# cxy1997/3D_adapt_auto_driving

Measured on AMD Instinct MI355X. Metric: KITTI scenes/s end-to-end eval_rcnn (joint RPN+RCNN, synthetic 16384-pt scenes), higher is better.
Workload: dtype f32; 1 GPU; BASELINE.json configs[2]: full PointRCNN RPN+RCNN inference, default.yaml shapes, random-init weights, batch=8 synthetic KITTI scenes x 16384 pts per GPU per step; scene=synth.scenes (SURVEY 8d: uniform clutter + ground + 10 dense cars), parallelism=scene-sharded x1, one final all_gather of detections, detections_gathered=652455, batch_slots=14, look_ahead=12, steps_per_launch=2

## Files before the change

### 3d_adapt_auto_driving_amd/csrc/fps_spec.hip

```cpp
#include "fps_common.hpp"
#include <stdlib.h>
#include <map>
#include <mutex>

namespace prcnn {



constexpr int FS_RMAX = 16;

__device__ __forceinline__ float fs_shfl(float v, int src, int wbase)
{
    const int index = (src & (WAVE - 1)) + wbase;
    return __int_as_float(__builtin_amdgcn_ds_bpermute(index << 2, __float_as_int(v)));
}

template <int PPT, int I = 0>
__device__ __forceinline__ void fs_pick3(const float (&px)[PPT], const float (&py)[PPT], const float (&pz)[PPT], int slot, int l,
                                         float &x, float &y, float &z)
{
    if (slot == I) {
        x = __int_as_float(__builtin_amdgcn_readlane(__float_as_int(px[I]), l));
        y = __int_as_float(__builtin_amdgcn_readlane(__float_as_int(py[I]), l));
        z = __int_as_float(__builtin_amdgcn_readlane(__float_as_int(pz[I]), l));
    } else if constexpr (I + 1 < PPT) {
        fs_pick3<PPT, I + 1>(px, py, pz, slot, l, x, y, z);
    }
}

template <int PPT>
__global__ __launch_bounds__(1024) void fps_spec_kernel(
    int n, int m, KeyCodec kc, const float *__restrict__ xyz, const int *__restrict__ perm,
    float *__restrict__ temp, int *__restrict__ idx, float *__restrict__ new_xyz, const int *__restrict__ rejected = nullptr)
{
    constexpr int SB = PPT == 16 ? 4 : (PPT == 8 ? 3 : 2);
    __shared__ unsigned long long s_vk[32];
    __shared__ float s_xyz[32][3];
    __shared__ float s_bound[16];
    __shared__ int s_rank[32], s_blk[32];
    const int b = blockIdx.x;
    if (rejected && rejected[b] == 0) return;
    const float *__restrict__ cloud = xyz + (long)b * n * 3;
    const int *__restrict__ order = perm + (long)b * n;
    float *__restrict__ mind = temp ? temp + (long)b * n : nullptr;
    int *__restrict__ sel = idx + (long)b * m;
    float *__restrict__ nxyz = new_xyz ? new_xyz + (long)b * m * 3 : nullptr;
    const int t = threadIdx.x, lane = t & 63, w = t >> 6;
    __builtin_amdgcn_s_setprio(3);

    float px[PPT], py[PPT], pz[PPT], pt[PPT];
    uint32_t pc[PPT];
    float bx0 = INFINITY, bx1 = -INFINITY, by0 = INFINITY, by1 = -INFINITY, bz0 = INFINITY, bz1 = -INFINITY;
#pragma unroll
    for (int i = 0; i < PPT; ++i) {
        const int s = w * (64 * PPT) + i * 64 + lane;
        float x0 = INFINITY, x1 = -INFINITY, y0 = INFINITY, y1 = -INFINITY, z0 = INFINITY, z1 = -INFINITY;
        if (s < n) {
            const int k = order[s];
            px[i] = cloud[3 * k]; py[i] = cloud[3 * k + 1]; pz[i] = cloud[3 * k + 2];
            pt[i] = mind ? mind[k] : 1e10f;
            pc[i] = (kc.encode(k) << SB) | (uint32_t)i;
            x0 = x1 = px[i]; y0 = y1 = py[i]; z0 = z1 = pz[i];
        } else {
            px[i] = py[i] = pz[i] = 0.f;
            pt[i] = -INFINITY;
            pc[i] = 0xffffffffu;
        }
#pragma unroll
        for (int d = 32; d >= 1; d >>= 1) {
            x0 = fmin_raw(x0, __shfl_xor(x0, d, 64)); x1 = fmax_raw(x1, __shfl_xor(x1, d, 64));
            y0 = fmin_raw(y0, __shfl_xor(y0, d, 64)); y1 = fmax_raw(y1, __shfl_xor(y1, d, 64));
            z0 = fmin_raw(z0, __shfl_xor(z0, d, 64)); z1 = fmax_raw(z1, __shfl_xor(z1, d, 64));
        }
        if (lane == i) { bx0 = x0; bx1 = x1; by0 = y0; by1 = y1; bz0 = z0; bz1 = z1; }
    }

    constexpr int GP = 64 / PPT;
    const int wbase = (int)__lane_id() & ~(WAVE - 1);
    bx0 = fs_shfl(bx0, lane & (PPT - 1), wbase); bx1 = fs_shfl(bx1, lane & (PPT - 1), wbase);
    by0 = fs_shfl(by0, lane & (PPT - 1), wbase); by1 = fs_shfl(by1, lane & (PPT - 1), wbase);
    bz0 = fs_shfl(bz0, lane & (PPT - 1), wbase); bz1 = fs_shfl(bz1, lane & (PPT - 1), wbase);
    unsigned long long touched = 0ull, etiles = ~0ull;
    float bound = INFINITY;
    auto box_mask = [&](float ox, float oy, float oz, bool live) __attribute__((always_inline)) {
        const float dx = fmax_raw(fmax_raw(bx0 - ox, ox - bx1), 0.f);
        const float dy = fmax_raw(fmax_raw(by0 - oy, oy - by1), 0.f);
        const float dz = fmax_raw(fmax_raw(bz0 - oz, oz - bz1), 0.f);
        const float lb = dx * dx + dy * dy + dz * dz;
        return __ballot(live && !(lb * 0.99999f >= bound));
    };
    auto update = [&](float ox, float oy, float oz, unsigned long long mask) __attribute__((always_inline)) {
        if (mask != 0ull) {
            touched |= mask & etiles;
            const pk_f32x2 o_x = {ox, ox}, o_y = {oy, oy}, o_z = {oz, oz};
            if (kc.hipcc) {
#pragma unroll
                for (int i = 0; i < PPT; i += 2)
                    if ((mask >> i) & 3ull) {
                        const pk_f32x2 dx = (pk_f32x2){px[i], px[i + 1]} - o_x, dy = (pk_f32x2){py[i], py[i + 1]} - o_y,
                                       dz = (pk_f32x2){pz[i], pz[i + 1]} - o_z;
                        const pk_f32x2 d = __builtin_elementwise_fma(dy, dy, dx * dx) + dz * dz;
                        pt[i] = fmin_raw(d.x, pt[i]); pt[i + 1] = fmin_raw(d.y, pt[i + 1]);
                    }
            } else {
#pragma unroll
                for (int i = 0; i < PPT; i += 2)
                    if ((mask >> i) & 3ull) {
                        const pk_f32x2 dx = (pk_f32x2){px[i], px[i + 1]} - o_x, dy = (pk_f32x2){py[i], py[i + 1]} - o_y,
                                       dz = (pk_f32x2){pz[i], pz[i + 1]} - o_z;
                        const pk_f32x2 d = (dx * dx + dy * dy) + dz * dz;
                        pt[i] = fmin_raw(d.x, pt[i]); pt[i + 1] = fmin_raw(d.y, pt[i + 1]);
                    }
            }
        }
    };
    if (t == 0) {
        sel[0] = 0;
        if (nxyz) { nxyz[0] = cloud[0]; nxyz[1] = cloud[1]; nxyz[2] = cloud[2]; }
    }
    if (t < 32) { s_rank[t] = 0; s_blk[t] = 0; }
    int j = 1;
    if (m > 1) {
        const float ox = cloud[0], oy = cloud[1], oz = cloud[2];
        update(ox, oy, oz, box_mask(ox, oy, oz, lane < PPT));
    }
    touched = ~0ull;
    while (j < m) {
        if (touched != 0ull) {
            float bv = -INFINITY, sv = -INFINITY;
#pragma unroll
            for (int i = 0; i < PPT; ++i) {
                sv = __builtin_amdgcn_fmed3f(bv, sv, pt[i]);
                bv = fmax_raw(bv, pt[i]);
            }
            uint32_t lk = 0xffffffffu;
#pragma unroll
            for (int i = 0; i < PPT; ++i) {
                const uint32_t c = pt[i] == bv ? pc[i] : 0xffffffffu;
                lk = c < lk ? c : lk;
            }
            const float v1 = wave_max_f32(bv);
            const uint32_t c1 = wave_min_u32(bv == v1 ? lk : 0xffffffffu);
            const unsigned long long m1 = __ballot(bv == v1 && lk == c1);
            const int l1 = m1 ? (int)__builtin_ctzll(m1) : 0;
            const float bv2 = lane == l1 ? -INFINITY : bv;
            const float v2 = wave_max_f32(bv2);
            const uint32_t c2 = wave_min_u32(bv2 == v2 ? lk : 0xffffffffu);
            const unsigned long long m2 = __ballot(lane != l1 && bv2 == v2 && lk == c2);
            const int l2 = m2 ? (int)__builtin_ctzll(m2) : l1;
            const float v3 = wave_max_f32((lane == l1 || lane == l2) ? -INFINITY : bv);
            const float s1 = __int_as_float(__builtin_amdgcn_readlane(__float_as_int(sv), l1));
            const float s2 = __int_as_float(__builtin_amdgcn_readlane(__float_as_int(sv), l2));
            const float wB = fmax_raw(v3, fmax_raw(s1, s2));
            bound = v1;
            const int sl1 = (int)(c1 & ((1u << SB) - 1u)), sl2 = (int)(c2 & ((1u << SB) - 1u));
            const bool has2 = m2 != 0ull && c2 != 0xffffffffu;
            etiles = (1ull << sl1) | (has2 ? (1ull << sl2) : 0ull);
            float x1 = 0.f, y1 = 0.f, z1 = 0.f, x2 = 0.f, y2 = 0.f, z2 = 0.f;
            fs_pick3<PPT>(px, py, pz, __builtin_amdgcn_readfirstlane(sl1), l1, x1, y1, z1);
            fs_pick3<PPT>(px, py, pz, __builtin_amdgcn_readfirstlane(sl2), l2, x2, y2, z2);
            const float ex = lane == 0 ? x1 : x2, ey = lane == 0 ? y1 : y2, ez = lane == 0 ? z1 : z2;
            if (lane < 2) {
                const float ev = lane == 0 ? v1 : (has2 ? v2 : -INFINITY);
                const uint32_t ek = lane == 0 ? (c1 == 0xffffffffu ? 0xffffffffu : (c1 >> SB)) : (has2 ? (c2 >> SB) : 0xffffffffu);
                s_vk[2 * w + lane] = pack_candidate(ev, ek);
                s_xyz[2 * w + lane][0] = ex; s_xyz[2 * w + lane][1] = ey; s_xyz[2 * w + lane][2] = ez;
                if (lane == 0) s_bound[w] = wB;
            }
        }
        lds_barrier();
        const int left = m - j;
        const int e = lane & 31, h = lane >> 5;
        const unsigned long long pke = s_vk[e];
        float cv; uint32_t ck;
        unpack_candidate(pke, cv, ck);
        const float cx = s_xyz[e][0], cy = s_xyz[e][1], cz = s_xyz[e][2];
        const float gB = wave_max_f32(lane < 16 ? s_bound[lane] : -INFINITY);
        {
            const int i = 2 * w + h;
            const unsigned long long pki = s_vk[i];
            float iv; uint32_t ik;
            unpack_candidate(pki, iv, ik);
            const float ix = s_xyz[i][0], iy = s_xyz[i][1], iz = s_xyz[i][2];
            const bool before = pke > pki;
            const float d = kc.hipcc ? fps_dist<true>(ix, iy, iz, cx, cy, cz) : sqdist3(ix, iy, iz, cx, cy, cz);
            const unsigned long long bb = __ballot(before), kb = __ballot(before && (d < iv));
            if (e == 0) {
                s_rank[i] = __popc((unsigned)(h ? (bb >> 32) : bb));
                s_blk[i] = (unsigned)(h ? (kb >> 32) : kb) != 0u;
            }
        }
        lds_barrier();
        const int rank = s_rank[e];
        const bool blocked = s_blk[e] != 0;
        const bool valid = !(ck == 0xffffffffu || !(cv > -1.0f));
        const bool pass = rank == 0 ? true : ((cv > gB) && (cv > 0.f) && valid && !blocked);
        const bool stop = !pass || (rank == 0 && !valid);
        int r = (int)wave_min_u32((stop && !(rank == 0)) ? (uint32_t)rank : ((rank == 0 && !valid) ? 1u : 32u));
        r = min(min(r, left), FS_RMAX);
        if (r < 1) r = 1;
        const float ox_ = valid ? cx : cloud[0], oy_ = valid ? cy : cloud[1], oz_ = valid ? cz : cloud[2];
        if (w == 0 && h == 0 && rank < r) {
            sel[j + rank] = valid ? kc.decode(ck) : 0;
            if (nxyz) { nxyz[3 * (j + rank)] = ox_; nxyz[3 * (j + rank) + 1] = oy_; nxyz[3 * (j + rank) + 2] = oz_; }
        }
        const int dst = (h == 0 && rank < FS_RMAX) ? 3 * rank : 63;
        const float rv = __int_as_float(__builtin_amdgcn_ds_permute(dst << 2, __float_as_int(ox_)) |
                                        __builtin_amdgcn_ds_permute(min(dst + 1, 63) << 2, __float_as_int(oy_)) |
                                        __builtin_amdgcn_ds_permute(min(dst + 2, 63) << 2, __float_as_int(oz_)));
        j += r;
        const int apply_n = j >= m ? r - 1 : r;
        touched = 0ull;
        for (int q0 = 0; q0 < apply_n; q0 += GP) {
            const int qg = q0 + lane / PPT;
            const int src = 3 * min(qg, FS_RMAX - 1);
            const float gx = fs_shfl(rv, src, wbase), gy = fs_shfl(rv, src + 1, wbase), gz = fs_shfl(rv, src + 2, wbase);
            const unsigned long long masks = box_mask(gx, gy, gz, qg < apply_n);
            if (masks == 0ull) continue;
#pragma unroll
            for (int g = 0; g < GP; ++g) {
                const unsigned long long mk = (masks >> (g * PPT)) & ((PPT == 64) ? ~0ull : ((1ull << PPT) - 1ull));
                if (mk != 0ull) {
                    const int q = q0 + g;
                    const float ox = __int_as_float(__builtin_amdgcn_readlane(__float_as_int(rv), 3 * q));
                    const float oy = __int_as_float(__builtin_amdgcn_readlane(__float_as_int(rv), 3 * q + 1));
                    const float oz = __int_as_float(__builtin_amdgcn_readlane(__float_as_int(rv), 3 * q + 2));
                    update(ox, oy, oz, mk);
                }
            }
        }
    }
    if (mind) {
#pragma unroll
        for (int i = 0; i < PPT; ++i)
            if (pc[i] != 0xffffffffu) mind[kc.decode(pc[i] >> SB)] = pt[i];
    }
}

struct Fps2Table {
    unsigned long long vk[2][64];
    float xyz[2][64][4];
    float bound[2][32];
    unsigned int sync;
    unsigned int pad[63];
};

__device__ __forceinline__ unsigned long long ld_agent_u64(const unsigned long long *p)
{
    return __hip_atomic_load(p, __ATOMIC_RELAXED, __HIP_MEMORY_SCOPE_AGENT);
}
__device__ __forceinline__ float ld_agent_f32(const float *p)
{
    return __int_as_float(__hip_atomic_load(reinterpret_cast<const int *>(p), __ATOMIC_RELAXED, __HIP_MEMORY_SCOPE_AGENT));
}

__device__ __forceinline__ void st_agent_u64(unsigned long long *p, unsigned long long v)
{
    __hip_atomic_store(p, v, __ATOMIC_RELAXED, __HIP_MEMORY_SCOPE_AGENT);
}
__device__ __forceinline__ void st_agent_f32(float *p, float v)
{
    __hip_atomic_store(reinterpret_cast<int *>(p), __float_as_int(v), __ATOMIC_RELAXED, __HIP_MEMORY_SCOPE_AGENT);
}

__global__ __launch_bounds__(1024) void fps_spec2_kernel(
    int nclouds, int n, int m, KeyCodec kc, const float *__restrict__ xyz, const int *__restrict__ perm,
    float *__restrict__ temp, int *__restrict__ idx, float *__restrict__ new_xyz, Fps2Table *__restrict__ tables)
{
    constexpr int PPT = 16, SB = 4, NE = 64;
    __shared__ unsigned long long s_vk[NE];
    __shared__ float s_xyz[NE][3];
    __shared__ float s_bound[32];
    __shared__ float s_res[64];
    __shared__ int s_rank[NE], s_blk[NE];
    __shared__ unsigned long long s_evk[32];
    __shared__ float s_exyz[32][3], s_eb[16];
    const int q_ = blockIdx.x;
    const int b = (q_ >> 4) * 8 + (q_ & 7), half = (q_ >> 3) & 1;
    if (b >= nclouds) return;
    const float *__restrict__ cloud = xyz + (long)b * n * 3;
    const int *__restrict__ order = perm + (long)b * n;
    float *__restrict__ mind = temp ? temp + (long)b * n : nullptr;
    int *__restrict__ sel = idx + (long)b * m;
    float *__restrict__ nxyz = new_xyz ? new_xyz + (long)b * m * 3 : nullptr;
    Fps2Table *__restrict__ tb = tables + b;
    const int t = threadIdx.x, lane = t & 63, w = t >> 6, gw = 16 * half + w;
    __builtin_amdgcn_s_setprio(3);

    float px[PPT], py[PPT], pz[PPT], pt[PPT];
    uint32_t pc[PPT];
    float bx0 = INFINITY, bx1 = -INFINITY, by0 = INFINITY, by1 = -INFINITY, bz0 = INFINITY, bz1 = -INFINITY;
#pragma unroll
    for (int i = 0; i < PPT; ++i) {
        const int s = gw * (64 * PPT) + i * 64 + lane;
        float x0 = INFINITY, x1 = -INFINITY, y0 = INFINITY, y1 = -INFINITY, z0 = INFINITY, z1 = -INFINITY;
        if (s < n) {
            const int k = order[s];
            px[i] = cloud[3 * k]; py[i] = cloud[3 * k + 1]; pz[i] = cloud[3 * k + 2];
            pt[i] = mind ? mind[k] : 1e10f;
            pc[i] = (kc.encode(k) << SB) | (uint32_t)i;
            x0 = x1 = px[i]; y0 = y1 = py[i]; z0 = z1 = pz[i];
        } else {
            px[i] = py[i] = pz[i] = 0.f;
            pt[i] = -INFINITY;
            pc[i] = 0xffffffffu;
        }
#pragma unroll
        for (int d = 32; d >= 1; d >>= 1) {
            x0 = fmin_raw(x0, __shfl_xor(x0, d, 64)); x1 = fmax_raw(x1, __shfl_xor(x1, d, 64));
            y0 = fmin_raw(y0, __shfl_xor(y0, d, 64)); y1 = fmax_raw(y1, __shfl_xor(y1, d, 64));
            z0 = fmin_raw(z0, __shfl_xor(z0, d, 64)); z1 = fmax_raw(z1, __shfl_xor(z1, d, 64));
        }
        if (lane == i) { bx0 = x0; bx1 = x1; by0 = y0; by1 = y1; bz0 = z0; bz1 = z1; }
    }
    constexpr int GP = 64 / PPT;
    const int wbase = (int)__lane_id() & ~(WAVE - 1);
    bx0 = fs_shfl(bx0, lane & (PPT - 1), wbase); bx1 = fs_shfl(bx1, lane & (PPT - 1), wbase);
    by0 = fs_shfl(by0, lane & (PPT - 1), wbase); by1 = fs_shfl(by1, lane & (PPT - 1), wbase);
    bz0 = fs_shfl(bz0, lane & (PPT - 1), wbase); bz1 = fs_shfl(bz1, lane & (PPT - 1), wbase);
    unsigned long long touched = 0ull;
    float bound = INFINITY;
    auto box_mask = [&](float ox, float oy, float oz, bool live) __attribute__((always_inline)) {
        const float dx = fmax_raw(fmax_raw(bx0 - ox, ox - bx1), 0.f);
        const float dy = fmax_raw(fmax_raw(by0 - oy, oy - by1), 0.f);
        const float dz = fmax_raw(fmax_raw(bz0 - oz, oz - bz1), 0.f);
        const float lb = dx * dx + dy * dy + dz * dz;
        return __ballot(live && !(lb * 0.99999f >= bound));
    };
    auto update = [&](float ox, float oy, float oz, unsigned long long mask) __attribute__((always_inline)) {
        if (mask != 0ull) {
            touched |= mask;
            const pk_f32x2 o_x = {ox, ox}, o_y = {oy, oy}, o_z = {oz, oz};
            if (kc.hipcc) {
#pragma unroll
                for (int i = 0; i < PPT; i += 2)
                    if ((mask >> i) & 3ull) {
                        const pk_f32x2 dx = (pk_f32x2){px[i], px[i + 1]} - o_x, dy = (pk_f32x2){py[i], py[i + 1]} - o_y,
                                       dz = (pk_f32x2){pz[i], pz[i + 1]} - o_z;
                        const pk_f32x2 d = __builtin_elementwise_fma(dy, dy, dx * dx) + dz * dz;
                        pt[i] = fmin_raw(d.x, pt[i]); pt[i + 1] = fmin_raw(d.y, pt[i + 1]);
                    }
            } else {
#pragma unroll
                for (int i = 0; i < PPT; i += 2)
                    if ((mask >> i) & 3ull) {
                        const pk_f32x2 dx = (pk_f32x2){px[i], px[i + 1]} - o_x, dy = (pk_f32x2){py[i], py[i + 1]} - o_y,
                                       dz = (pk_f32x2){pz[i], pz[i + 1]} - o_z;
                        const pk_f32x2 d = (dx * dx + dy * dy) + dz * dz;
                        pt[i] = fmin_raw(d.x, pt[i]); pt[i + 1] = fmin_raw(d.y, pt[i + 1]);
                    }
            }
        }
    };
    if (t == 0 && half == 0) {
        sel[0] = 0;
        if (nxyz) { nxyz[0] = cloud[0]; nxyz[1] = cloud[1]; nxyz[2] = cloud[2]; }
    }
    if (t < NE) { s_rank[t] = 0; s_blk[t] = 0; }
    int j = 1;
    if (m > 1) {
        const float ox = cloud[0], oy = cloud[1], oz = cloud[2];
        update(ox, oy, oz, box_mask(ox, oy, oz, lane < PPT));
    }
    touched = ~0ull;
    unsigned int round = 0;
    while (j < m) {
        if (touched != 0ull) {
            float bv = -INFINITY, sv = -INFINITY;
#pragma unroll
            for (int i = 0; i < PPT; ++i) {
                sv = __builtin_amdgcn_fmed3f(bv, sv, pt[i]);
                bv = fmax_raw(bv, pt[i]);
            }
            uint32_t lk = 0xffffffffu;
#pragma unroll
            for (int i = 0; i < PPT; ++i) {
                const uint32_t c = pt[i] == bv ? pc[i] : 0xffffffffu;
                lk = c < lk ? c : lk;
            }
            const float v1 = wave_max_f32(bv);
            const uint32_t c1 = wave_min_u32(bv == v1 ? lk : 0xffffffffu);
            const unsigned long long m1 = __ballot(bv == v1 && lk == c1);
            const int l1 = m1 ? (int)__builtin_ctzll(m1) : 0;
            const float bv2 = lane == l1 ? -INFINITY : bv;
            const float v2 = wave_max_f32(bv2);
            const uint32_t c2 = wave_min_u32(bv2 == v2 ? lk : 0xffffffffu);
            const unsigned long long m2 = __ballot(lane != l1 && bv2 == v2 && lk == c2);
            const int l2 = m2 ? (int)__builtin_ctzll(m2) : l1;
            const float v3 = wave_max_f32((lane == l1 || lane == l2) ? -INFINITY : bv);
            const float s1 = __int_as_float(__builtin_amdgcn_readlane(__float_as_int(sv), l1));
            const float s2 = __int_as_float(__builtin_amdgcn_readlane(__float_as_int(sv), l2));
            const float e_b = fmax_raw(v3, fmax_raw(s1, s2));
            bound = v1;
            const int sl1 = (int)(c1 & ((1u << SB) - 1u)), sl2 = (int)(c2 & ((1u << SB) - 1u));
            const bool has2 = m2 != 0ull && c2 != 0xffffffffu;
            float x1 = 0.f, y1 = 0.f, z1 = 0.f, x2 = 0.f, y2 = 0.f, z2 = 0.f;
            fs_pick3<PPT>(px, py, pz, __builtin_amdgcn_readfirstlane(sl1), l1, x1, y1, z1);
            fs_pick3<PPT>(px, py, pz, __builtin_amdgcn_readfirstlane(sl2), l2, x2, y2, z2);
            const float ev = lane == 0 ? v1 : (has2 ? v2 : -INFINITY);
            const uint32_t ek = lane == 0 ? (c1 == 0xffffffffu ? 0xffffffffu : (c1 >> SB)) : (has2 ? (c2 >> SB) : 0xffffffffu);
            if (lane < 2) {
                s_evk[2 * w + lane] = pack_candidate(ev, ek);
                s_exyz[2 * w + lane][0] = lane == 0 ? x1 : x2; s_exyz[2 * w + lane][1] = lane == 0 ? y1 : y2; s_exyz[2 * w + lane][2] = lane == 0 ? z1 : z2;
                if (lane == 0) s_eb[w] = e_b;
            }
        }
        const int par = (int)(round & 1u);
        if (lane < 2) {
            const int e = 2 * gw + lane, le = 2 * w + lane;
            st_agent_u64(&tb->vk[par][e], s_evk[le]);
            st_agent_f32(&tb->xyz[par][e][0], s_exyz[le][0]); st_agent_f32(&tb->xyz[par][e][1], s_exyz[le][1]);
            st_agent_f32(&tb->xyz[par][e][2], s_exyz[le][2]);
            if (lane == 0) st_agent_f32(&tb->bound[par][gw], s_eb[w]);
        }
        asm volatile("s_waitcnt vmcnt(0)" ::: "memory");
        __syncthreads();
        if (t == 0) {
            __hip_atomic_fetch_add(&tb->sync, 1u, __ATOMIC_RELEASE, __HIP_MEMORY_SCOPE_AGENT);
            const unsigned int want = 2u * (round + 1u);
            const long long t0 = wall_clock64();
            while (__hip_atomic_load(&tb->sync, __ATOMIC_ACQUIRE, __HIP_MEMORY_SCOPE_AGENT) < want) {
                __builtin_amdgcn_s_sleep(1);
                if (wall_clock64() - t0 > 400000000ll) __builtin_trap();
            }
        }
        __syncthreads();
        if (t < NE) {
            s_vk[t] = ld_agent_u64(&tb->vk[par][t]);
            s_xyz[t][0] = ld_agent_f32(&tb->xyz[par][t][0]);
            s_xyz[t][1] = ld_agent_f32(&tb->xyz[par][t][1]);
            s_xyz[t][2] = ld_agent_f32(&tb->xyz[par][t][2]);
            if (t < 32) s_bound[t] = ld_agent_f32(&tb->bound[par][t]);
        }
        __syncthreads();
        const int left = m - j;
        const int i = lane;
        const unsigned long long pki = s_vk[i];
        float cv; uint32_t ck;
        unpack_candidate(pki, cv, ck);
        const float cx = s_xyz[i][0], cy = s_xyz[i][1], cz = s_xyz[i][2];
        {
            int rk = 0;
            bool bl = false;
#pragma unroll 1
            for (int u = 0; u < 4; ++u) {
                const int e = 4 * w + u;
                const unsigned long long pke = s_vk[e];
                const float ex = s_xyz[e][0], ey = s_xyz[e][1], ez = s_xyz[e][2];
                const bool before = pke > pki;
                const float d = kc.hipcc ? fps_dist<true>(cx, cy, cz, ex, ey, ez) : sqdist3(cx, cy, cz, ex, ey, ez);
                rk += before ? 1 : 0;
                bl = bl || (before && (d < cv));
            }
            if (rk) atomicAdd(&s_rank[i], rk);
            if (bl) atomicOr(&s_blk[i], 1);
        }
        lds_barrier();
        if (w == 0) {
            const int rank = s_rank[i];
            const bool blocked = s_blk[i] != 0;
            const float gB = wave_max_f32(lane < 32 ? s_bound[lane] : -INFINITY);
            const bool valid = !(ck == 0xffffffffu || !(cv > -1.0f));
            const bool pass = rank == 0 ? true : ((cv > gB) && (cv > 0.f) && valid && !blocked);
            const bool stop = !pass || (rank == 0 && !valid);
            int r = (int)wave_min_u32((stop && !(rank == 0)) ? (uint32_t)rank : ((rank == 0 && !valid) ? 1u : 64u));
            r = min(min(r, left), FS_RMAX);
            if (r < 1) r = 1;
            if (rank < r) {
                const bool v0 = valid;
                const float ox = v0 ? cx : cloud[0], oy = v0 ? cy : cloud[1], oz = v0 ? cz : cloud[2];
                s_res[1 + 3 * rank] = ox; s_res[2 + 3 * rank] = oy; s_res[3 + 3 * rank] = oz;
                if (half == 0) {
                    sel[j + rank] = valid ? kc.decode(ck) : 0;
                    if (nxyz) { nxyz[3 * (j + rank)] = ox; nxyz[3 * (j + rank) + 1] = oy; nxyz[3 * (j + rank) + 2] = oz; }
                }
            }
            s_rank[i] = 0; s_blk[i] = 0;
            if (lane == 0) s_res[0] = __int_as_float(r);
        }
        lds_barrier();
        const float rv = s_res[lane];
        const int r = __builtin_amdgcn_readfirstlane(__float_as_int(rv));
        j += r;
        const int apply_n = j >= m ? r - 1 : r;
        touched = 0ull;
        for (int q0 = 0; q0 < apply_n; q0 += GP) {
            const int qg = q0 + lane / PPT;
            const int src = 1 + 3 * min(qg, FS_RMAX - 1);
            const float gx = fs_shfl(rv, src, wbase), gy = fs_shfl(rv, src + 1, wbase), gz = fs_shfl(rv, src + 2, wbase);
            const unsigned long long masks = box_mask(gx, gy, gz, qg < apply_n);
            if (masks == 0ull) continue;
#pragma unroll
            for (int g = 0; g < GP; ++g) {
                const unsigned long long mk = (masks >> (g * PPT)) & ((1ull << PPT) - 1ull);
                if (mk != 0ull) {
                    const int q = q0 + g;
                    const float ox = __int_as_float(__builtin_amdgcn_readlane(__float_as_int(rv), 1 + 3 * q));
                    const float oy = __int_as_float(__builtin_amdgcn_readlane(__float_as_int(rv), 2 + 3 * q));
                    const float oz = __int_as_float(__builtin_amdgcn_readlane(__float_as_int(rv), 3 + 3 * q));
                    update(ox, oy, oz, mk);
                }
            }
        }
        ++round;
    }
    if (mind) {
#pragma unroll
        for (int i = 0; i < PPT; ++i)
            if (pc[i] != 0xffffffffu) mind[kc.decode(pc[i] >> SB)] = pt[i];
    }
}

static size_t fps_lds_pad()
{
    static const size_t pad = (size_t)(getenv("PRCNN_FPS_LDS_PAD") ? atoi(getenv("PRCNN_FPS_LDS_PAD")) : 84) * 1024;
    return pad;
}

int fps2_capacity()
{
    static std::mutex mu;
    static std::map<int, int> cache;
    const size_t pad = fps_lds_pad();
    int dev = 0;
    if (hipGetDevice(&dev) != hipSuccess) { (void)hipGetLastError(); return 0; }
    std::lock_guard<std::mutex> lock(mu);
    auto it = cache.find(dev);
    if (it != cache.end()) return it->second;
    int cap = 0, per_cu = 0, cus = 0;
    if (ensure_dynamic_lds((const void *)prcnn::fps_spec2_kernel, pad, "furthest_point_sampling(two workgroups)") == PRCNN_OK &&
        hipOccupancyMaxActiveBlocksPerMultiprocessor(&per_cu, (const void *)prcnn::fps_spec2_kernel, 1024, pad) == hipSuccess &&
        hipDeviceGetAttribute(&cus, hipDeviceAttributeMultiprocessorCount, dev) == hipSuccess)
        cap = per_cu * cus;
    else
        (void)hipGetLastError();
    if (const char *e = getenv("PRCNN_FPS2_CAPACITY")) cap = atoi(e);
    cache[dev] = cap;
    return cap;
}

int launch_fps_spec2(int b, int n, int m, KeyCodec kc, const float *xyz, float *temp, int *idx, float *new_xyz, hipStream_t st)
{
    int *perm = (int *)scratch_for(st, (size_t)b * n * sizeof(int), 1);
    Fps2Table *tables = (Fps2Table *)scratch_for(st, (size_t)b * sizeof(Fps2Table), 13);
    if (!perm || !tables) { set_error("fps: cannot allocate the ordering / exchange scratch"); return PRCNN_ELAUNCH; }
    launch_fps_order(b, n, xyz, perm, nullptr, st);
    if (hipMemsetAsync(tables, 0, (size_t)b * sizeof(Fps2Table), st) != hipSuccess) {
        (void)hipGetLastError();
        set_error("fps: cannot reset the exchange tables");
        return PRCNN_ELAUNCH;
    }
    const int per = (fps2_capacity() / 2 / 16) * 8;
    for (int off = 0; off < b; off += per) {
        const int nb = b - off < per ? b - off : per;
        const unsigned grid = (unsigned)((nb + 7) / 8) * 16u;
        hipLaunchKernelGGL(fps_spec2_kernel, dim3(grid), dim3(1024), fps_lds_pad(), st, nb, n, m, kc, xyz + (size_t)off * n * 3, perm + (size_t)off * n,
                           temp ? temp + (size_t)off * n : nullptr, idx + (size_t)off * m, new_xyz ? new_xyz + (size_t)off * m * 3 : nullptr,
                           tables + off);
    }
    return check_launch("furthest_point_sampling(two workgroups)");
}

int launch_fps_spec(int b, int n, int m, KeyCodec kc, const float *xyz, float *temp, int *idx, float *new_xyz, const int *rejected, hipStream_t st)
{
    int *perm = (int *)scratch_for(st, (size_t)b * n * sizeof(int), 1);
    if (!perm) { set_error("fps: cannot allocate ordering scratch"); return PRCNN_ELAUNCH; }
    launch_fps_order(b, n, xyz, perm, rejected, st);
    const size_t pad = b <= 128 ? fps_lds_pad() : 0;
    const void *ss[3] = {(const void *)fps_spec_kernel<4>, (const void *)fps_spec_kernel<8>, (const void *)fps_spec_kernel<16>};
    if (pad)
        for (const void *k : ss) {
            const int rc = ensure_dynamic_lds(k, pad, "furthest_point_sampling(speculative)");
            if (rc != PRCNN_OK) return rc;
        }
    if (n <= 4096) hipLaunchKernelGGL((fps_spec_kernel<4>), dim3(b), dim3(1024), pad, st, n, m, kc, xyz, perm, temp, idx, new_xyz, rejected);
    else if (n <= 8192) hipLaunchKernelGGL((fps_spec_kernel<8>), dim3(b), dim3(1024), pad, st, n, m, kc, xyz, perm, temp, idx, new_xyz, rejected);
    else hipLaunchKernelGGL((fps_spec_kernel<16>), dim3(b), dim3(1024), pad, st, n, m, kc, xyz, perm, temp, idx, new_xyz, rejected);
    return check_launch("furthest_point_sampling(speculative)");
}

}
```

### profiles/fps_stamps.py

```python
import ctypes, importlib, os, subprocess, sys
import numpy as np

ROOT = os.path.dirname(os.path.dirname(os.path.abspath(__file__)))
CSRC = os.path.join(ROOT, "3d_adapt_auto_driving_amd", "csrc")
EXP = os.path.join(ROOT, "profiles", "_exp")
LIB = os.path.join(EXP, "libprcnn_hip_fps_stamps.so")
FLAGS = "--offload-arch=gfx950 -O3 -std=c++17 -fPIC -ffp-contract=off -fno-fast-math".split()
NPH = 8


def instrument():
    s = open(os.path.join(CSRC, "fps_spec.hip")).read()
    s = s.replace('#include "fps_common.hpp"', '#include "%s/fps_common.hpp"' % CSRC)
    a = s.index("template <int PPT>\n__global__ __launch_bounds__(1024) void fps_spec_kernel(")
    b = s.index("// The speculative kernel for 16384 < n <= 32768")
    k = s[a:b]

    def put(old, new):
        nonlocal k
        assert k.count(old) == 1, old[:70]
        k = k.replace(old, new)
    put("    while (j < m) {\n", "    unsigned long long acc_[%d] = {0}, t_prev_ = __builtin_amdgcn_s_memtime();\n#define PH(i) { const unsigned long long n_ = __builtin_amdgcn_s_memtime(); acc_[i] += n_ - t_prev_; t_prev_ = n_; }\n    while (j < m) {\n        acc_[7] += 1;\n" % NPH)
    put("        lds_barrier();                                                // A: the table is complete\n", "        PH(0)\n        lds_barrier();                                                // A: the table is complete\n        PH(1)\n")
    put("        lds_barrier();                                                // A2: every entry has its rank\n", "        PH(2)\n        lds_barrier();                                                // A2: every entry has its rank\n        PH(3)\n")
    put("        // ---- 4. running minima against this round's pivots (the last pick of the whole run does not update them: sampling_gpu.cu)\n", "        PH(4)\n        PH(5)\n        // ---- 4. running minima against this round's pivots (the last pick of the whole run does not update them: sampling_gpu.cu)\n")
    put("    if (mind) {\n#pragma unroll\n        for (int i = 0; i < PPT; ++i)\n            if (pc[i] != 0xffffffffu) mind[kc.decode(pc[i] >> SB)] = pt[i];\n    }\n}",
        "    if (mind) {\n#pragma unroll\n        for (int i = 0; i < PPT; ++i)\n            if (pc[i] != 0xffffffffu) mind[kc.decode(pc[i] >> SB)] = pt[i];\n    }\n"
        "    if (blockIdx.x == 0 && lane == 0) for (int i = 0; i < %d; ++i) g_fps_acc[w * %d + i] = acc_[i];\n}" % (NPH, NPH))
    put("                    update(ox, oy, oz, mk);\n                }\n            }\n        }\n    }\n", "                    update(ox, oy, oz, mk);\n                }\n            }\n        }\n        PH(6)\n    }\n")
    k = "__device__ unsigned long long g_fps_acc[16 * %d];\n" % NPH + k
    s = s[:a] + k + s[b:]
    s += ('\nextern "C" int prcnn_debug_fps_acc(unsigned long long *dst)\n{\n    return (int)hipMemcpyFromSymbol(dst, HIP_SYMBOL(prcnn::g_fps_acc), '
          'sizeof(unsigned long long) * 16 * %d);\n}\n' % NPH)
    return s


def build():
    os.makedirs(EXP, exist_ok=True)
    subprocess.check_call(["make", "-C", CSRC])
    src = os.path.join(EXP, "fps_stamps.hip")
    open(src, "w").write(instrument())
    obj = os.path.join(EXP, "fps_stamps.o")
    subprocess.check_call(["/opt/rocm/bin/hipcc"] + FLAGS + ["-c", src, "-o", obj])
    objs = [os.path.join(CSRC, "build", f) for f in sorted(os.listdir(os.path.join(CSRC, "build"))) if f.endswith(".o") and f != "fps_spec.o"]
    subprocess.check_call(["/opt/rocm/bin/hipcc", "--offload-arch=gfx950", "-shared", "-fPIC", "-o", LIB, obj] + objs)
    print("built", LIB)


def run(kind):
    import torch
    sys.path.insert(0, ROOT)
    L = importlib.import_module("3d_adapt_auto_driving_amd._lib")
    L.LIB_PATH = LIB
    pkg = importlib.import_module("3d_adapt_auto_driving_amd"); sys.path.insert(0, pkg.DROPIN_DIR)
    import pointnet2_cuda as P
    synth = importlib.import_module("3d_adapt_auto_driving_amd.synth")
    dev = torch.device("cuda", 0)
    xyz = torch.from_numpy((synth.lidar_scenes if kind == "lidar" else synth.scenes)(8, 16384, seed0=0)).to(dev)
    n, m = 16384, 4096
    temp = torch.empty((8, n), device=dev); idx = torch.empty((8, m), dtype=torch.int32, device=dev)
    for _ in range(3):
        temp.fill_(1e10); P.furthest_point_sampling_wrapper(8, n, m, xyz, temp, idx)
    torch.cuda.synchronize()
    buf = (ctypes.c_ulonglong * (16 * NPH))()
    lib = ctypes.CDLL(LIB)
    assert lib.prcnn_debug_fps_acc(buf) == 0
    a = np.array(buf, dtype=np.float64).reshape(16, NPH)
    rounds = a[:, 7]
    print("%s scenes, cloud 0, 16384 -> 4096: %d rounds; s_memtime cycles per round by wave" % (kind, int(rounds[0])))
    print("wave | rebuild+publish | wait A | pairs | wait A2 | verdict + permute (every wave, round 6) | - | updates | sum")
    for w in range(16):
        v = a[w, :7] / rounds[w]
        print("%4d | " % w + " | ".join("%7.1f" % x for x in v) + " | %7.1f" % v.sum())
    v = (a[:, :7] / rounds[:, None]).mean(0)
    print("mean | " + " | ".join("%7.1f" % x for x in v) + " | %7.1f" % v.sum())


if __name__ == "__main__":
    if sys.argv[1] == "build":
        build()
    else:
        run(sys.argv[2] if len(sys.argv) > 2 else "uniform")
```

Before: 9047 scenes/s.

## Cull FPS pivot updates with per-wave bounding box and drop permute broadcasts

Each wave now keeps a bounding box over all its points and tests every accepted pivot against it. Only pivots that could lower some running minimum in the wave are iterated, serially, and each is read with readlane or a uniform LDS load. This replaces the ds_permute/bpermute broadcast and the grouped per-tile box tests. It also adds a fast path in the key tie-break that skips a wave-min reduction when exactly one lane holds the maximum, and turns the slot pick into a binary search. The risk is that serial per-pivot iteration is slower when most pivots hit the wave.

```diff
diff --git a/3d_adapt_auto_driving_amd/csrc/fps_spec.hip b/3d_adapt_auto_driving_amd/csrc/fps_spec.hip
--- a/3d_adapt_auto_driving_amd/csrc/fps_spec.hip
+++ b/3d_adapt_auto_driving_amd/csrc/fps_spec.hip
@@ -9,22 +9,33 @@
 
 constexpr int FS_RMAX = 16;
 
-__device__ __forceinline__ float fs_shfl(float v, int src, int wbase)
-{
-    const int index = (src & (WAVE - 1)) + wbase;
-    return __int_as_float(__builtin_amdgcn_ds_bpermute(index << 2, __float_as_int(v)));
-}
-
-template <int PPT, int I = 0>
+__device__ __forceinline__ float fs_uniform(float v)
+{
+    return __int_as_float(__builtin_amdgcn_readfirstlane(__float_as_int(v)));
+}
+__device__ __forceinline__ float fs_readlane(float v, int l)
+{
+    return __int_as_float(__builtin_amdgcn_readlane(__float_as_int(v), l));
+}
+
+__device__ __forceinline__ void fs_key_of(bool in, bool also, uint32_t lk, uint32_t &c, unsigned long long &m)
+{
+    const unsigned long long a = __ballot(in);
+    if (__popcll(a) == 1) c = (uint32_t)__builtin_amdgcn_readlane((int)lk, (int)__builtin_ctzll(a));
+    else c = wave_min_u32(in ? lk : 0xffffffffu);
+    m = a & __ballot(also && lk == c);
+}
+
+template <int PPT, int LO = 0, int N = PPT>
 __device__ __forceinline__ void fs_pick3(const float (&px)[PPT], const float (&py)[PPT], const float (&pz)[PPT], int slot, int l,
                                          float &x, float &y, float &z)
 {
-    if (slot == I) {
-        x = __int_as_float(__builtin_amdgcn_readlane(__float_as_int(px[I]), l));
-        y = __int_as_float(__builtin_amdgcn_readlane(__float_as_int(py[I]), l));
-        z = __int_as_float(__builtin_amdgcn_readlane(__float_as_int(pz[I]), l));
-    } else if constexpr (I + 1 < PPT) {
-        fs_pick3<PPT, I + 1>(px, py, pz, slot, l, x, y, z);
+    if constexpr (N == 1) {
+        x = fs_readlane(px[LO], l); y = fs_readlane(py[LO], l); z = fs_readlane(pz[LO], l);
+    } else if (slot < LO + N / 2) {
+        fs_pick3<PPT, LO, N / 2>(px, py, pz, slot, l, x, y, z);
+    } else {
+        fs_pick3<PPT, LO + N / 2, N / 2>(px, py, pz, slot, l, x, y, z);
     }
 }
 
@@ -51,6 +62,7 @@
     float px[PPT], py[PPT], pz[PPT], pt[PPT];
     uint32_t pc[PPT];
     float bx0 = INFINITY, bx1 = -INFINITY, by0 = INFINITY, by1 = -INFINITY, bz0 = INFINITY, bz1 = -INFINITY;
+    float wx0 = INFINITY, wx1 = -INFINITY, wy0 = INFINITY, wy1 = -INFINITY, wz0 = INFINITY, wz1 = -INFINITY;
 #pragma unroll
     for (int i = 0; i < PPT; ++i) {
         const int s = w * (64 * PPT) + i * 64 + lane;
@@ -73,13 +85,11 @@
             z0 = fmin_raw(z0, __shfl_xor(z0, d, 64)); z1 = fmax_raw(z1, __shfl_xor(z1, d, 64));
         }
         if (lane == i) { bx0 = x0; bx1 = x1; by0 = y0; by1 = y1; bz0 = z0; bz1 = z1; }
-    }
-
-    constexpr int GP = 64 / PPT;
-    const int wbase = (int)__lane_id() & ~(WAVE - 1);
-    bx0 = fs_shfl(bx0, lane & (PPT - 1), wbase); bx1 = fs_shfl(bx1, lane & (PPT - 1), wbase);
-    by0 = fs_shfl(by0, lane & (PPT - 1), wbase); by1 = fs_shfl(by1, lane & (PPT - 1), wbase);
-    bz0 = fs_shfl(bz0, lane & (PPT - 1), wbase); bz1 = fs_shfl(bz1, lane & (PPT - 1), wbase);
+        wx0 = fmin_raw(wx0, x0); wx1 = fmax_raw(wx1, x1); wy0 = fmin_raw(wy0, y0); wy1 = fmax_raw(wy1, y1);
+        wz0 = fmin_raw(wz0, z0); wz1 = fmax_raw(wz1, z1);
+    }
+    wx0 = fs_uniform(wx0); wx1 = fs_uniform(wx1); wy0 = fs_uniform(wy0); wy1 = fs_uniform(wy1); wz0 = fs_uniform(wz0); wz1 = fs_uniform(wz1);
+
     unsigned long long touched = 0ull, etiles = ~0ull;
     float bound = INFINITY;
     auto box_mask = [&](float ox, float oy, float oz, bool live) __attribute__((always_inline)) {
@@ -89,6 +99,13 @@
         const float lb = dx * dx + dy * dy + dz * dz;
         return __ballot(live && !(lb * 0.99999f >= bound));
     };
+    auto wave_hit = [&](float ox, float oy, float oz) __attribute__((always_inline)) {
+        const float dx = fmax_raw(fmax_raw(wx0 - ox, ox - wx1), 0.f);
+        const float dy = fmax_raw(fmax_raw(wy0 - oy, oy - wy1), 0.f);
+        const float dz = fmax_raw(fmax_raw(wz0 - oz, oz - wz1), 0.f);
+        const float lb = dx * dx + dy * dy + dz * dz;
+        return !(lb * 0.99999f >= bound);
+    };
     auto update = [&](float ox, float oy, float oz, unsigned long long mask) __attribute__((always_inline)) {
         if (mask != 0ull) {
             touched |= mask & etiles;
@@ -140,13 +157,13 @@
                 lk = c < lk ? c : lk;
             }
             const float v1 = wave_max_f32(bv);
-            const uint32_t c1 = wave_min_u32(bv == v1 ? lk : 0xffffffffu);
-            const unsigned long long m1 = __ballot(bv == v1 && lk == c1);
+            uint32_t c1; unsigned long long m1;
+            fs_key_of(bv == v1, true, lk, c1, m1);
             const int l1 = m1 ? (int)__builtin_ctzll(m1) : 0;
             const float bv2 = lane == l1 ? -INFINITY : bv;
             const float v2 = wave_max_f32(bv2);
-            const uint32_t c2 = wave_min_u32(bv2 == v2 ? lk : 0xffffffffu);
-            const unsigned long long m2 = __ballot(lane != l1 && bv2 == v2 && lk == c2);
+            uint32_t c2; unsigned long long m2;
+            fs_key_of(bv2 == v2, lane != l1, lk, c2, m2);
             const int l2 = m2 ? (int)__builtin_ctzll(m2) : l1;
             const float v3 = wave_max_f32((lane == l1 || lane == l2) ? -INFINITY : bv);
             const float s1 = __int_as_float(__builtin_amdgcn_readlane(__float_as_int(sv), l1));
@@ -190,10 +207,11 @@
                 s_blk[i] = (unsigned)(h ? (kb >> 32) : kb) != 0u;
             }
         }
+        const bool valid = !(ck == 0xffffffffu || !(cv > -1.0f));
+        const bool hit = wave_hit(cx, cy, cz) || !valid;
         lds_barrier();
         const int rank = s_rank[e];
         const bool blocked = s_blk[e] != 0;
-        const bool valid = !(ck == 0xffffffffu || !(cv > -1.0f));
         const bool pass = rank == 0 ? true : ((cv > gB) && (cv > 0.f) && valid && !blocked);
         const bool stop = !pass || (rank == 0 && !valid);
         int r = (int)wave_min_u32((stop && !(rank == 0)) ? (uint32_t)rank : ((rank == 0 && !valid) ? 1u : 32u));
@@ -204,30 +222,15 @@
             sel[j + rank] = valid ? kc.decode(ck) : 0;
             if (nxyz) { nxyz[3 * (j + rank)] = ox_; nxyz[3 * (j + rank) + 1] = oy_; nxyz[3 * (j + rank) + 2] = oz_; }
         }
-        const int dst = (h == 0 && rank < FS_RMAX) ? 3 * rank : 63;
-        const float rv = __int_as_float(__builtin_amdgcn_ds_permute(dst << 2, __float_as_int(ox_)) |
-                                        __builtin_amdgcn_ds_permute(min(dst + 1, 63) << 2, __float_as_int(oy_)) |
-                                        __builtin_amdgcn_ds_permute(min(dst + 2, 63) << 2, __float_as_int(oz_)));
         j += r;
         const int apply_n = j >= m ? r - 1 : r;
         touched = 0ull;
-        for (int q0 = 0; q0 < apply_n; q0 += GP) {
-            const int qg = q0 + lane / PPT;
-            const int src = 3 * min(qg, FS_RMAX - 1);
-            const float gx = fs_shfl(rv, src, wbase), gy = fs_shfl(rv, src + 1, wbase), gz = fs_shfl(rv, src + 2, wbase);
-            const unsigned long long masks = box_mask(gx, gy, gz, qg < apply_n);
-            if (masks == 0ull) continue;
-#pragma unroll
-            for (int g = 0; g < GP; ++g) {
-                const unsigned long long mk = (masks >> (g * PPT)) & ((PPT == 64) ? ~0ull : ((1ull << PPT) - 1ull));
-                if (mk != 0ull) {
-                    const int q = q0 + g;
-                    const float ox = __int_as_float(__builtin_amdgcn_readlane(__float_as_int(rv), 3 * q));
-                    const float oy = __int_as_float(__builtin_amdgcn_readlane(__float_as_int(rv), 3 * q + 1));
-                    const float oz = __int_as_float(__builtin_amdgcn_readlane(__float_as_int(rv), 3 * q + 2));
-                    update(ox, oy, oz, mk);
-                }
-            }
+        unsigned mine = (unsigned)__ballot(h == 0 && rank < apply_n && hit);
+        while (mine != 0u) {
+            const int l = __builtin_ctz(mine);
+            mine &= mine - 1u;
+            const float ox = fs_readlane(ox_, l), oy = fs_readlane(oy_, l), oz = fs_readlane(oz_, l);
+            update(ox, oy, oz, box_mask(ox, oy, oz, lane < PPT));
         }
     }
     if (mind) {
@@ -290,6 +293,7 @@
     float px[PPT], py[PPT], pz[PPT], pt[PPT];
     uint32_t pc[PPT];
     float bx0 = INFINITY, bx1 = -INFINITY, by0 = INFINITY, by1 = -INFINITY, bz0 = INFINITY, bz1 = -INFINITY;
+    float wx0 = INFINITY, wx1 = -INFINITY, wy0 = INFINITY, wy1 = -INFINITY, wz0 = INFINITY, wz1 = -INFINITY;
 #pragma unroll
     for (int i = 0; i < PPT; ++i) {
         const int s = gw * (64 * PPT) + i * 64 + lane;
@@ -312,12 +316,10 @@
             z0 = fmin_raw(z0, __shfl_xor(z0, d, 64)); z1 = fmax_raw(z1, __shfl_xor(z1, d, 64));
         }
         if (lane == i) { bx0 = x0; bx1 = x1; by0 = y0; by1 = y1; bz0 = z0; bz1 = z1; }
-    }
-    constexpr int GP = 64 / PPT;
-    const int wbase = (int)__lane_id() & ~(WAVE - 1);
-    bx0 = fs_shfl(bx0, lane & (PPT - 1), wbase); bx1 = fs_shfl(bx1, lane & (PPT - 1), wbase);
-    by0 = fs_shfl(by0, lane & (PPT - 1), wbase); by1 = fs_shfl(by1, lane & (PPT - 1), wbase);
-    bz0 = fs_shfl(bz0, lane & (PPT - 1), wbase); bz1 = fs_shfl(bz1, lane & (PPT - 1), wbase);
+        wx0 = fmin_raw(wx0, x0); wx1 = fmax_raw(wx1, x1); wy0 = fmin_raw(wy0, y0); wy1 = fmax_raw(wy1, y1);
+        wz0 = fmin_raw(wz0, z0); wz1 = fmax_raw(wz1, z1);
+    }
+    wx0 = fs_uniform(wx0); wx1 = fs_uniform(wx1); wy0 = fs_uniform(wy0); wy1 = fs_uniform(wy1); wz0 = fs_uniform(wz0); wz1 = fs_uniform(wz1);
     unsigned long long touched = 0ull;
     float bound = INFINITY;
     auto box_mask = [&](float ox, float oy, float oz, bool live) __attribute__((always_inline)) {
@@ -327,6 +329,13 @@
         const float lb = dx * dx + dy * dy + dz * dz;
         return __ballot(live && !(lb * 0.99999f >= bound));
     };
+    auto wave_hit = [&](float ox, float oy, float oz) __attribute__((always_inline)) {
+        const float dx = fmax_raw(fmax_raw(wx0 - ox, ox - wx1), 0.f);
+        const float dy = fmax_raw(fmax_raw(wy0 - oy, oy - wy1), 0.f);
+        const float dz = fmax_raw(fmax_raw(wz0 - oz, oz - wz1), 0.f);
+        const float lb = dx * dx + dy * dy + dz * dz;
+        return !(lb * 0.99999f >= bound);
+    };
     auto update = [&](float ox, float oy, float oz, unsigned long long mask) __attribute__((always_inline)) {
         if (mask != 0ull) {
             touched |= mask;
@@ -379,13 +388,13 @@
                 lk = c < lk ? c : lk;
             }
             const float v1 = wave_max_f32(bv);
-            const uint32_t c1 = wave_min_u32(bv == v1 ? lk : 0xffffffffu);
-            const unsigned long long m1 = __ballot(bv == v1 && lk == c1);
+            uint32_t c1; unsigned long long m1;
+            fs_key_of(bv == v1, true, lk, c1, m1);
             const int l1 = m1 ? (int)__builtin_ctzll(m1) : 0;
             const float bv2 = lane == l1 ? -INFINITY : bv;
             const float v2 = wave_max_f32(bv2);
-            const uint32_t c2 = wave_min_u32(bv2 == v2 ? lk : 0xffffffffu);
-            const unsigned long long m2 = __ballot(lane != l1 && bv2 == v2 && lk == c2);
+            uint32_t c2; unsigned long long m2;
+            fs_key_of(bv2 == v2, lane != l1, lk, c2, m2);
             const int l2 = m2 ? (int)__builtin_ctzll(m2) : l1;
             const float v3 = wave_max_f32((lane == l1 || lane == l2) ? -INFINITY : bv);
             const float s1 = __int_as_float(__builtin_amdgcn_readlane(__float_as_int(sv), l1));
@@ -479,28 +488,18 @@
             if (lane == 0) s_res[0] = __int_as_float(r);
         }
         lds_barrier();
-        const float rv = s_res[lane];
-        const int r = __builtin_amdgcn_readfirstlane(__float_as_int(rv));
+        const int r = __float_as_int(s_res[0]);
+        const int q3 = 1 + 3 * min(lane, FS_RMAX - 1);
+        const float ox_ = s_res[q3], oy_ = s_res[q3 + 1], oz_ = s_res[q3 + 2];
         j += r;
         const int apply_n = j >= m ? r - 1 : r;
         touched = 0ull;
-        for (int q0 = 0; q0 < apply_n; q0 += GP) {
-            const int qg = q0 + lane / PPT;
-            const int src = 1 + 3 * min(qg, FS_RMAX - 1);
-            const float gx = fs_shfl(rv, src, wbase), gy = fs_shfl(rv, src + 1, wbase), gz = fs_shfl(rv, src + 2, wbase);
-            const unsigned long long masks = box_mask(gx, gy, gz, qg < apply_n);
-            if (masks == 0ull) continue;
-#pragma unroll
-            for (int g = 0; g < GP; ++g) {
-                const unsigned long long mk = (masks >> (g * PPT)) & ((1ull << PPT) - 1ull);
-                if (mk != 0ull) {
-                    const int q = q0 + g;
-                    const float ox = __int_as_float(__builtin_amdgcn_readlane(__float_as_int(rv), 1 + 3 * q));
-                    const float oy = __int_as_float(__builtin_amdgcn_readlane(__float_as_int(rv), 2 + 3 * q));
-                    const float oz = __int_as_float(__builtin_amdgcn_readlane(__float_as_int(rv), 3 + 3 * q));
-                    update(ox, oy, oz, mk);
-                }
-            }
+        unsigned mine = (unsigned)__ballot(lane < apply_n && wave_hit(ox_, oy_, oz_));
+        while (mine != 0u) {
+            const int l = __builtin_ctz(mine);
+            mine &= mine - 1u;
+            const float ox = fs_uniform(s_res[1 + 3 * l]), oy = fs_uniform(s_res[2 + 3 * l]), oz = fs_uniform(s_res[3 + 3 * l]);
+            update(ox, oy, oz, box_mask(ox, oy, oz, lane < PPT));
         }
         ++round;
     }
diff --git a/profiles/fps_stamps.py b/profiles/fps_stamps.py
--- a/profiles/fps_stamps.py
+++ b/profiles/fps_stamps.py
@@ -27,7 +27,7 @@
     put("    if (mind) {\n#pragma unroll\n        for (int i = 0; i < PPT; ++i)\n            if (pc[i] != 0xffffffffu) mind[kc.decode(pc[i] >> SB)] = pt[i];\n    }\n}",
         "    if (mind) {\n#pragma unroll\n        for (int i = 0; i < PPT; ++i)\n            if (pc[i] != 0xffffffffu) mind[kc.decode(pc[i] >> SB)] = pt[i];\n    }\n"
         "    if (blockIdx.x == 0 && lane == 0) for (int i = 0; i < %d; ++i) g_fps_acc[w * %d + i] = acc_[i];\n}" % (NPH, NPH))
-    put("                    update(ox, oy, oz, mk);\n                }\n            }\n        }\n    }\n", "                    update(ox, oy, oz, mk);\n                }\n            }\n        }\n        PH(6)\n    }\n")
+    put("            update(ox, oy, oz, box_mask(ox, oy, oz, lane < PPT));\n        }\n    }\n", "            update(ox, oy, oz, box_mask(ox, oy, oz, lane < PPT));\n        }\n        PH(6)\n    }\n")
     k = "__device__ unsigned long long g_fps_acc[16 * %d];\n" % NPH + k
     s = s[:a] + k + s[b:]
     s += ('\nextern "C" int prcnn_debug_fps_acc(unsigned long long *dst)\n{\n    return (int)hipMemcpyFromSymbol(dst, HIP_SYMBOL(prcnn::g_fps_acc), '
@@ -68,7 +68,7 @@
     a = np.array(buf, dtype=np.float64).reshape(16, NPH)
     rounds = a[:, 7]
     print("%s scenes, cloud 0, 16384 -> 4096: %d rounds; s_memtime cycles per round by wave" % (kind, int(rounds[0])))
-    print("wave | rebuild+publish | wait A | pairs | wait A2 | verdict + permute (every wave, round 6) | - | updates | sum")
+    print("wave | rebuild+publish | wait A | pairs | wait A2 | verdict + own pivots (every wave, round 7) | - | updates | sum")
     for w in range(16):
         v = a[w, :7] / rounds[w]
         print("%4d | " % w + " | ".join("%7.1f" % x for x in v) + " | %7.1f" % v.sum())
```

New measurement: 9158 scenes/s, median of 6. 1.2% higher.
